# Jun-CEN/Open-World-Semantic-Segmentation

Hardware: AMD Instinct MI355X
Metric: images/sec train-step, DeepLabV3+R101 768x768 bs=16; % HBM & MFMA roofline (higher is better)
Workload: dtype f16x2

## Files before the change

include/dmlnet_hip.h:

```cpp
#ifndef DMLNET_HIP_H
#define DMLNET_HIP_H

#include <stdint.h>

#ifdef __cplusplus
extern "C" {
#endif

#define DML_ABI_VERSION 6

enum { DML_F32 = 0, DML_BF16 = 1 };
enum { DML_EINVAL = -1, DML_EALIGN = -2, DML_EUNSUPPORTED = -3 };

int dml_abi_version(void);
const char* dml_target_arch(void);

typedef struct DmlConvDesc {
    const void* x;
    const void* w;
    void* y;
    const float* bias;
    float* stats;
    int32_t B, Hi, Wi, C, ldx;
    int32_t Ho, Wo, N, ldy;
// ... 45 lines not shown
                 int32_t layout, float* work, int32_t amax_known, void* stream);

typedef struct DmlH2Desc {
    const float* x;
    void* planes;
    float* work;
    int64_t rows, plane_stride;
    int32_t C, ld, ldp, layout;
} DmlH2Desc;
int dml_h2_split_table(const DmlH2Desc* table_device, int count, void* stream);

typedef struct DmlWgradDesc {
    const void* x;
    const void* dy;
    float* dw;
    int32_t B, Hi, Wi, C, ldx;
    int32_t Ho, Wo, N, ldy;
    int32_t R, S, stride, dil, pad;
    int32_t dtype;
    int32_t splitk;
    int32_t Cm;
    float* ws;
    int64_t ws_elems;
    int32_t f32_split;
    int32_t reserved;
    const void* x_planes;
    const void* dy_planes;
    const float* x_unscale;
    const float* dy_unscale;
    int64_t x_plane_stride, dy_plane_stride;
} DmlWgradDesc;

int dml_conv_wgrad(const DmlWgradDesc* d, void* stream);

int dml_conv_wgrad_group_eligible(const DmlWgradDesc* d);
int dml_conv_wgrad_group(const DmlWgradDesc* const* descs, int n, float* ws, int64_t ws_elems, void* stream);

int dml_prep_weight(const float* w_master, void* w, void* wt, int N, int RS, int Cm, int Cp, int dtype,
                    void* stream);
typedef struct DmlPrepDesc {
    const float* src;
    void* w;
    void* wt;
    int32_t N, RS, Cm, Cp;
    int32_t w_tiled, wt_tiled;
} DmlPrepDesc;
int dml_prep_weights(const DmlPrepDesc* descs_device, int count, int dtype, void* stream);
int dml_unpad_wgrad(const float* src, float* dst, int N, int RS, int Cm, int Cp, void* stream);
int dml_bias_grad(const void* dy, float* db, int64_t M, int N, int ldy, int dtype, void* stream);
int dml_bias_grad_ws(const void* dy, float* db, int64_t M, int N, int ldy, int dtype, float* ws, int64_t ws_elems, void* stream);

int dml_pack_input(const float* x_nchw, void* y_nhwc, int B, int C, int H, int W, int Cp, int dtype,
                   void* stream);
int dml_pack_input_s2d(const float* x_nchw, float* x2, int B, int C, int H, int W, void* stream);
int dml_s2d_weights(const float* w, float* w2, int N, int k, int C, void* stream);
int dml_gather_taps(const float* src, float* dst, int rows, int taps_src, int n, int ntaps, int t0, int t1, int t2, int t3,
                    void* stream);
int dml_s2d_wgrad(const float* dw2, float* dw, int N, int k, int C, void* stream);

int dml_bn_finalize(float* partials, int64_t M, int N, int stat_rows, const float* gamma, const float* beta,
                    float* running_mean, float* running_var, float momentum, float eps,
                    float* scale, float* shift, float* save_mean, float* save_invstd, void* stream);
int dml_bn_moments(float* partials, int64_t M, int N, int stat_rows, double* moments, void* stream);
int dml_bn_finalize_moments(const double* moments, int ranks, int64_t M_each, int N, const float* gamma,
                            const float* beta, float* running_mean, float* running_var, float momentum,
                            float eps, float* scale, float* shift, float* save_mean, float* save_invstd,
// ... 258 lines not shown
```

open-world-semantic-segmentation_amd/csrc/bn.hip:

```cpp
#include "common.h"
#include <cstdlib>

namespace {

struct Moments {
    double n, mean, m2;
};
__device__ __forceinline__ void merge(Moments& a, double nb, double meanb, double m2b) {
    if (nb <= 0.0) return;
    const double n = a.n + nb;
    const double d = meanb - a.mean;
    a.mean += d * (nb / n);
    a.m2 += m2b + d * d * (a.n * nb / n);
    a.n = n;
}

constexpr int FIN_CH = 4, FIN_SL = 64;
__device__ __forceinline__ double shfl_xor_f64(double v, int mask) {
    const long long b = __double_as_longlong(v);
    const int lo = __shfl_xor((int)(b & 0xffffffffll), mask), hi = __shfl_xor((int)(b >> 32), mask);
    return __longlong_as_double(((long long)hi << 32) | (unsigned int)lo);
}

__device__ __forceinline__ float h2_words_max(const float* __restrict__ words, float* sh4) {
// ... 1197 lines not shown
            const uint32_t am = *reinterpret_cast<const uint32_t*>(argmax + o);
#pragma unroll
            for (int u = 0; u < 2; ++u) {
                const int r = 2 * by + u - (2 * yo - 1);
                if (r < 0 || r > 2) continue;
#pragma unroll
                for (int t = 0; t < 2; ++t) {
                    const int s = 2 * bx + t - (2 * xo - 1);
                    if (s < 0 || s > 2) continue;
#pragma unroll
                    for (int q = 0; q < 4; ++q) acc[u][t][q] += (((am >> (q * 8)) & 0xffu) == (uint32_t)(r * 3 + s)) ? g[q] : 0.f;
                }
            }
        }
    }
#pragma unroll
    for (int u = 0; u < 2; ++u) {
#pragma unroll
        for (int t = 0; t < 2; ++t) {
            const int yi = 2 * by + u, xi = 2 * bx + t;
            if (yi >= H || xi >= W) continue;
            const uint32_t bits = mask[(((int64_t)b * H + yi) * W + xi) * (C / 4) + cv];
#pragma unroll
            for (int q = 0; q < 4; ++q) acc[u][t][q] = ((bits >> q) & 1u) != 0 ? acc[u][t][q] : 0.f;
        }
    }
}

__device__ __forceinline__ void stem_pixel_grad(const float* __restrict__ dp, const uint8_t* __restrict__ argmax, uint32_t bits, int b,
                                                int yi, int xi, int C, int Ho, int Wo, int cv, float (&acc)[4]) {
#pragma unroll
    for (int q = 0; q < 4; ++q) acc[q] = 0.f;
    const int by = yi >> 1, bx = xi >> 1, u = yi & 1, t = xi & 1;
#pragma unroll
    for (int dyo = 0; dyo < 2; ++dyo) {
        const int yo = by + dyo, r = u + 1 - 2 * dyo;
        if (yo >= Ho || r < 0) continue;
#pragma unroll
        for (int dxo = 0; dxo < 2; ++dxo) {
            const int xo = bx + dxo, sc = t + 1 - 2 * dxo;
            if (xo >= Wo || sc < 0) continue;
            const int64_t o = (((int64_t)b * Ho + yo) * Wo + xo) * C + cv * 4;
            float g[4];
            Vec16<float>::load(dp + o, g);
            const uint32_t am = *reinterpret_cast<const uint32_t*>(argmax + o);
#pragma unroll
            for (int q = 0; q < 4; ++q) acc[q] += (((am >> (q * 8)) & 0xffu) == (uint32_t)(r * 3 + sc)) ? g[q] : 0.f;
        }
    }
#pragma unroll
    for (int q = 0; q < 4; ++q) acc[q] = ((bits >> q) & 1u) != 0 ? acc[q] : 0.f;
}

__global__ __launch_bounds__(256) void stem_bwd_reduce_kernel(
    const float* __restrict__ dp, const uint8_t* __restrict__ argmax, const uint8_t* __restrict__ mask, const float* __restrict__ y,
    const float* __restrict__ save_mean, const float* __restrict__ save_invstd, float* __restrict__ partials, int B, int H, int W,
    int C, int ldy, int Ho, int Wo, int rows_per_block, int chv, int rt, uint32_t* __restrict__ gmax) {
    __shared__ float sh[256 * 2 * 4];
    uint32_t gmx = 0;
    const int NV = C / 4;
    const int64_t M = (int64_t)B * H * W;
    const int col = threadIdx.x % chv, rl = threadIdx.x / chv;
    const int v = blockIdx.y * chv + col;
    const bool active = rl < rt && v < NV;
    float sg[4], sgx[4];
#pragma unroll
    for (int q = 0; q < 4; ++q) { sg[q] = 0.f; sgx[q] = 0.f; }
    if (active) {
        const int c = v * 4;
        float mu[4], is[4];
#pragma unroll
        for (int q = 0; q < 4; ++q) { mu[q] = save_mean[c + q]; is[q] = save_invstd[c + q]; }
        const int64_t r0 = (int64_t)blockIdx.x * rows_per_block;
        const int64_t r1 = min(M, r0 + rows_per_block);
        constexpr int U = 2;
        for (int64_t m0 = r0 + rl; m0 < r1; m0 += (int64_t)rt * U) {
            float g[U][4], yy[U][4];
#pragma unroll
            for (int u = 0; u < U; ++u) {
                const int64_t m = m0 + (int64_t)u * rt;
                if (m < r1) {
// ... 537 lines not shown
```

open-world-semantic-segmentation_amd/csrc/conv_igemm.hip:

```cpp
#include "common.h"
#include "conv_choice.h"
#include <cstdlib>

namespace {

constexpr int BK = 32;
constexpr int NTHREADS = 256;

typedef __bf16 mfma_bf16x8 __attribute__((ext_vector_type(8)));

struct ConvArgs {
    const void* x;
    const void* w;
    void* y;
    const float* bias;
    float* stats;
    int B, Hi, Wi, C, ldx;
    int Ho, Wo, N, ldy;
    int R, S, stride, dil, pad;
    int M, Ktot;
    int y_f32, accum;
    int nblk_n, nblk_m;
    FastDiv div_wo, div_howo, div_c;
    float* unused0_;
// ... 2193 lines not shown
        mm(0, 2); split_store(y_reg[1], Ys, lds_off(1)); split_store(x_reg[1], Xs, lds_off(1)); load_row(t + 2, 1);
        mm(1, 1); split_store(y_reg[2], Ys, lds_off(2)); split_store(x_reg[2], Xs, lds_off(2)); load_row(t + 2, 2);
        mm(1, 0); split_store(y_reg[3], Ys, lds_off(3)); split_store(x_reg[3], Xs, lds_off(3)); load_row(t + 2, 3);
        mm(0, 1);
        mm(0, 0);
#pragma unroll
        for (int q = 0; q < 64; ++q) {
            __builtin_amdgcn_sched_group_barrier(0x008, 1, 0);
            __builtin_amdgcn_sched_group_barrier(0x002, LIN ? 3 : 4, 0);
            __builtin_amdgcn_sched_group_barrier(0x200, 1, 0);
            if (q % 8 == 7) __builtin_amdgcn_sched_group_barrier(0x020, 1, 0);
        }
        __syncthreads();
    }
#pragma unroll
    for (int i = 0; i < NT; ++i)
#pragma unroll
        for (int q = 0; q < 4; ++q) {
            const int n = n0 + wn * 64 + i * 16 + lq * 4 + q;
            if (n >= a.N) continue;
#pragma unroll
            for (int j = 0; j < MT; ++j) {
                const int k = kc0 + wk * 64 + j * 16 + lr;
                if (k < a.Ktot) {
                    if (a.ws != nullptr)
                        a.ws[((int64_t)split * a.N + n) * a.Ktot + k] = acc[i][j][q];
                    else
                        atomicAdd(a.dw + (int64_t)n * a.Ktot + k, acc[i][j][q]);
                }
            }
        }
}

constexpr int WGW_NST = 3, WGW_NLD = 3;
constexpr int WGW_TN = 128, WGW_TK = 256;
constexpr int WGW_YROW = WGW_TN * 2, WGW_XROW = WGW_TK * 2;
constexpr int WGW_YPL = 32 * WGW_YROW, WGW_XPL = 32 * WGW_XROW;
constexpr int WGW_SB = 2 * WGW_YPL + 2 * WGW_XPL;

template <bool LIN, int LW>
__device__ __forceinline__ void wgrad_ws_loader(const WgradArgs& a, const uint32_t x_bytes, const uint32_t dy_bytes, char* smem,
                                                uint32_t* ready, uint32_t* consumed, const int lane, const int nitems, const int ntile) {
    constexpr int NLD = WGW_NLD, NST = WGW_NST, NG = 24, MYG = NG / NLD;
    constexpr uint32_t OOB = 0x80000000u;
    const u32x4_ws rs_x = ws_make_rsrc(a.x_planes, x_bytes + a.x_plane_bytes), rs_y = ws_make_rsrc(a.dy_planes, dy_bytes + a.dy_plane_bytes);
    const uint32_t lds0 = (uint32_t)(uintptr_t)smem;
    const int tiles_total = (a.M + BK - 1) / BK;
    uint32_t g = 0, pub = 0;
    for (int item = xcd_remap(blockIdx.x, gridDim.x); item < nitems; item += (int)gridDim.x) {
        const int split = item / ntile, tile_id = item - split * ntile;
        const int blk_n = tile_id % a.nblk_n, blk_k = tile_id / a.nblk_n;
        const int n0 = blk_n * WGW_TN, kc0 = blk_k * WGW_TK;
        const int tile_beg = split * a.slab_tiles, tile_end = min(tiles_total, tile_beg + a.slab_tiles);
        const int m_end = min(a.M, tile_end * BK);
        int row[MYG], colb[MYG], dyo[MYG], dxo[MYG];
        bool cok[MYG];
#pragma unroll
        for (int q = 0; q < MYG; ++q) {
            const int gi = q * NLD + LW;
            if (gi < 8) {
                row[q] = gi * 4 + (lane >> 4);
                const int gch = (lane & 15) ^ (2 * (row[q] & 7));
                const int n = n0 + gch * 8;
                cok[q] = n < a.N;
                colb[q] = n * 2;
                dyo[q] = dxo[q] = 0;
// ... 903 lines not shown
    switch (c.family) {
    case cc::WGRAD_BIG:
        hipLaunchKernelGGL(conv_wgrad_big_kernel<WGRAD_DEPTH>, grid, block, 0, st, a, c.x_bytes, c.dy_bytes);
        break;
    case cc::WGRAD_WS:
        if (c.lin) hipLaunchKernelGGL(conv_wgrad_ws_kernel<true>, grid, block, 0, st, a, c.x_bytes, c.dy_bytes, c.nitems);
        else hipLaunchKernelGGL(conv_wgrad_ws_kernel<false>, grid, block, 0, st, a, c.x_bytes, c.dy_bytes, c.nitems);
        break;
    case cc::WGRAD_H2:
        if (c.lin) hipLaunchKernelGGL(conv_wgrad_h2_kernel<true>, grid, block, 0, st, a, c.x_bytes, c.dy_bytes);
        else hipLaunchKernelGGL(conv_wgrad_h2_kernel<false>, grid, block, 0, st, a, c.x_bytes, c.dy_bytes);
        break;
    case cc::WGRAD_N64:
        hipLaunchKernelGGL(conv_wgrad_n64_kernel, grid, block, 0, st, a);
        break;
    case cc::WGRAD_X3:
        if (c.lin) hipLaunchKernelGGL(conv_wgrad_x3_kernel<true>, grid, block, 0, st, a, c.x_bytes, c.dy_bytes);
        else hipLaunchKernelGGL(conv_wgrad_x3_kernel<false>, grid, block, 0, st, a, c.x_bytes, c.dy_bytes);
        break;
    default:
        if (c.elem_bytes == 2) hipLaunchKernelGGL(conv_wgrad_kernel<bf16_t>, grid, block, 0, st, a);
        else hipLaunchKernelGGL(conv_wgrad_kernel<float>, grid, block, 0, st, a);
        break;
    }
    for (int i = 0; i < c.nreduce; ++i) {
        const cc::ReduceLaunch& r = c.reduce[i];
        hipLaunchKernelGGL(wgrad_reduce_kernel, dim3(r.grid_x, r.grid_y), dim3(r.block), 0, st, d->ws, d->dw, r.splits, c.nrs, c.cm, d->C,
                           r.slab_stride, r.fold_only);
    }
    DML_LAUNCH_CHECK();
    return 0;
}

extern "C" int dml_conv_wgrad_group_eligible(const DmlWgradDesc* d) { return cc::wgrad_big_eligible(d, true) ? 1 : 0; }

extern "C" int dml_conv_wgrad_group(const DmlWgradDesc* const* descs, int n, float* ws, int64_t ws_elems, void* stream) {
    cc::WgradGroupChoice c;
    const int rc = cc::wgrad_group_choose(descs, n, ws, ws_elems, &c);
    if (rc) return rc;
    WgradGroup g;
    ReduceGroup r;
    g.njobs = r.njobs = n;
    g.start[0] = 0;
    for (int j = 0; j < n; ++j) {
        const DmlWgradDesc* d = descs[j];
        WgradArgs& a = g.job[j];
        fill_wgrad_args(a, d, false);
        a.nblk_n = c.nblk_n[j]; a.nblk_k = c.nblk_k[j]; a.slab_tiles = c.slab_tiles[j];
        a.ws = ws + c.ws_off[j];
        g.xb[j] = c.x_bytes[j]; g.yb[j] = c.dy_bytes[j];
        g.start[j + 1] = c.start[j + 1];
        r.ws[j] = a.ws; r.dw[j] = d->dw; r.splits[j] = c.splitk[j]; r.Cm[j] = c.cm[j]; r.Cp[j] = d->C;
        r.NRS[j] = c.nrs[j];
    }
    hipStream_t st = static_cast<hipStream_t>(stream);
    hipLaunchKernelGGL(conv_wgrad_group_kernel<WGRAD_DEPTH>, dim3(c.grid), dim3(c.block), 0, st, g);
    hipLaunchKernelGGL(wgrad_reduce_group_kernel, dim3(c.rgrid_x, c.rgrid_y), dim3(c.rblock), 0, st, r);
    DML_LAUNCH_CHECK();
    return 0;
}
```

open-world-semantic-segmentation_amd/csrc/plan_exec.hip:

```cpp
#include "common.h"

#include <cstring>
#include <tuple>
#include <utility>

namespace {

template <class T> struct Unpack {
    static T get(uint64_t w) {
        if constexpr (std::is_pointer<T>::value) {
            return reinterpret_cast<T>(static_cast<uintptr_t>(w));
        } else if constexpr (std::is_same<T, float>::value) {
            const uint32_t lo = (uint32_t)w;
            float f;
            std::memcpy(&f, &lo, 4);
            return f;
        } else if constexpr (std::is_same<T, double>::value) {
            double d;
            std::memcpy(&d, &w, 8);
            return d;
        } else {
            return static_cast<T>(static_cast<int64_t>(w));
        }
    }
};

template <class R, class... Args, size_t... I>
int invoke(R (*f)(Args...), const uint64_t* w, void* st, std::index_sequence<I...>) {
    using Tup = std::tuple<Args...>;
    return (int)f(Unpack<std::tuple_element_t<I, Tup>>::get(w[I])..., st);
}
template <class R, class... Args> int thunk_call(R (*f)(Args...), const uint64_t* w, void* st) {
    return invoke(f, w, st, std::make_index_sequence<sizeof...(Args) - 1>{});
}
template <class R, class... Args> constexpr int arity(R (*)(Args...)) { return (int)sizeof...(Args) - 1; }

struct Entry {
    const char* name;
    int (*run)(const uint64_t*, void*);
    int nargs;
};

#define DML_ENTRY(fn) {#fn, [](const uint64_t* w, void* st) -> int { return thunk_call(&fn, w, st); }, arity(&fn)}

const Entry kEntries[] = {
    DML_ENTRY(dml_conv_igemm),
    DML_ENTRY(dml_conv_wgrad),
    DML_ENTRY(dml_conv_wgrad_group),
    DML_ENTRY(dml_prep_weight),
    DML_ENTRY(dml_prep_weights),
    DML_ENTRY(dml_unpad_wgrad),
    DML_ENTRY(dml_bias_grad),
    DML_ENTRY(dml_bias_grad_ws),
    DML_ENTRY(dml_pack_input),
    DML_ENTRY(dml_pack_input_s2d),
    DML_ENTRY(dml_s2d_weights),
    DML_ENTRY(dml_s2d_wgrad),
    DML_ENTRY(dml_bn_finalize),
    DML_ENTRY(dml_bn_moments),
    DML_ENTRY(dml_bn_finalize_moments),
    DML_ENTRY(dml_bn_bwd_sums),
    DML_ENTRY(dml_bn_bwd_coef),
    DML_ENTRY(dml_bn_stats),
    DML_ENTRY(dml_bn_eval_coeffs),
    DML_ENTRY(dml_bn_eval_coeffs_table),
    DML_ENTRY(dml_bn_apply),
    DML_ENTRY(dml_bn_bwd_reduce),
    DML_ENTRY(dml_bn_bwd_finalize),
    DML_ENTRY(dml_bn_bwd_apply),
    DML_ENTRY(dml_maxpool3x3s2_fwd),
    DML_ENTRY(dml_maxpool3x3s2_bwd),
    DML_ENTRY(dml_global_avgpool_fwd),
    DML_ENTRY(dml_broadcast_hw),
    DML_ENTRY(dml_reduce_hw),
    DML_ENTRY(dml_reduce_hw_f32),
    DML_ENTRY(dml_avgpool_bwd_add),
    DML_ENTRY(dml_avgpool_bwd_set),
    DML_ENTRY(dml_bilinear_fwd),
    DML_ENTRY(dml_bilinear_bwd),
    DML_ENTRY(dml_proto_dist_fwd),
    DML_ENTRY(dml_upsample_dist_fwd),
// ... 131 lines not shown
```

open-world-semantic-segmentation_amd/dmlnet/_lib.py:

```python
from __future__ import annotations

import ctypes as C
import os

_HERE = os.path.dirname(os.path.abspath(__file__))
LIB_PATH = os.environ.get("DML_LIB_PATH") or os.path.join(_HERE, "libdmlnet_hip.so")

DML_F32, DML_BF16 = 0, 1
STAT_ROWS = 64
LOSS_BLOCKS = 2048
FOCAL_PARTIALS = 3 * 2048
DISTILL_PARTIALS = 2 * 2048
OPEN_SWEEP_SPAN = 2048
OPEN_SWEEP_MAX_BLOCKS = 512
OPEN_SWEEP_MAX_T, OPEN_SWEEP_MAX_CLASSES, OPEN_SWEEP_MAX_OUT = 12, 33, 8


def metric_work_doubles(K, C):
    return 2048 * (2 + K * (C + 1))


c_p = C.c_void_p
c_i = C.c_int
c_i64 = C.c_int64
# ... 66 lines not shown
                ("op", C.c_int32 * 3), ("factor", C.c_float * 3)]


class ResizeScale(C.Structure):
    _fields_ = [("out", c_p), ("hbounds", c_p), ("hcoef", c_p), ("vbounds", c_p), ("vcoef", c_p),
                ("Hs", C.c_int32), ("Ws", C.c_int32), ("kh", C.c_int32), ("kv", C.c_int32),
                ("band_rows", C.c_int32), ("lds_rows", C.c_int32)]


RESIZE_MAX_SCALES = 8


class PredictHead(C.Structure):
    _fields_ = [("e", c_p), ("C", C.c_int32), ("K", C.c_int32), ("ld", C.c_int32), ("novel_id", C.c_int32)]


PREDICT_MAX_HEADS = 4
REC_MAX_SCALES = 8


class ScaleWindow(C.Structure):
    _fields_ = [("hbounds", C.c_int32), ("hcoef", C.c_int32), ("vbounds", C.c_int32), ("vcoef", C.c_int32),
                ("lrow", C.c_int32), ("lcol", C.c_int32), ("kh", C.c_int32), ("kv", C.c_int32)]


_PROTOS = {
    "dml_abi_version": (c_i, []),
    "dml_target_arch": (C.c_char_p, []),
    "dml_conv_igemm": (c_i, [C.POINTER(ConvDesc), c_p]),
    "dml_conv_stat_rows": (c_i, [C.POINTER(ConvDesc)]),
    "dml_h2_split_table": (c_i, [c_p, c_i, c_p]),
    "dml_h2_split": (c_i, [c_p, c_i64, c_i, c_i, c_p, c_i64, c_i, c_i, c_p, c_i, c_p]),
    "dml_conv_wgrad": (c_i, [C.POINTER(WgradDesc), c_p]),
    "dml_prep_weight": (c_i, [c_p, c_p, c_p, c_i, c_i, c_i, c_i, c_i, c_p]),
    "dml_prep_weights": (c_i, [c_p, c_i, c_i, c_p]),
    "dml_unpad_wgrad": (c_i, [c_p, c_p, c_i, c_i, c_i, c_i, c_p]),
    "dml_bias_grad": (c_i, [c_p, c_p, c_i64, c_i, c_i, c_i, c_p]),
    "dml_bias_grad_ws": (c_i, [c_p, c_p, c_i64, c_i, c_i, c_i, c_p, c_i64, c_p]),
    "dml_pack_input": (c_i, [c_p, c_p, c_i, c_i, c_i, c_i, c_i, c_i, c_p]),
    "dml_pack_input_s2d": (c_i, [c_p, c_p, c_i, c_i, c_i, c_i, c_p]),
    "dml_s2d_weights": (c_i, [c_p, c_p, c_i, c_i, c_i, c_p]),
    "dml_s2d_wgrad": (c_i, [c_p, c_p, c_i, c_i, c_i, c_p]),
    "dml_gather_taps": (c_i, [c_p, c_p, c_i, c_i, c_i, c_i, c_i, c_i, c_i, c_i, c_p]),
    "dml_bn_finalize": (c_i, [c_p, c_i64, c_i, c_i, c_p, c_p, c_p, c_p, c_f, c_f, c_p, c_p, c_p, c_p, c_p]),
    "dml_bn_moments": (c_i, [c_p, c_i64, c_i, c_i, c_p, c_p]),
    "dml_bn_finalize_moments": (c_i, [c_p, c_i, c_i64, c_i, c_p, c_p, c_p, c_p, c_f, c_f, c_p, c_p, c_p, c_p, c_p]),
    "dml_bn_bwd_sums": (c_i, [c_p, c_i, c_i, c_p, c_p, c_p, c_p]),
    "dml_bn_bwd_coef": (c_i, [c_p, c_i64, c_i, c_p, c_p, c_p, c_p, c_p]),
    "dml_bn_stats": (c_i, [c_p, c_p, c_i64, c_i, c_i, c_i, c_p]),
    "dml_bn_eval_coeffs": (c_i, [c_p, c_p, c_p, c_p, c_f, c_p, c_p, c_i, c_p]),
    "dml_bn_eval_coeffs_table": (c_i, [c_p, c_i, c_p]),
    "dml_bn_apply": (c_i, [c_p, c_p, c_p, c_p, c_p, c_p, c_p, c_i64, c_i, c_i, c_i, c_i, c_i, c_i, c_f, C.c_uint64, c_p,
                           c_p, c_i64, c_i, c_p, c_i64, c_p, c_p]),
    "dml_bn_bwd_reduce": (c_i, [c_p, c_p, c_p, c_p, c_p, c_p, c_p, c_i64, c_i, c_i, c_i, c_i, c_i, c_f, c_i,
                                C.POINTER(c_i), c_p, c_p]),
    "dml_bn_bwd_finalize": (c_i, [c_p, c_i, c_i64, c_i, c_p, c_p, c_p, c_p, c_p, c_p, c_p]),
    "dml_bn_bwd_apply": (c_i, [c_p, c_p, c_p, c_p, c_p, c_p, c_p, c_i64, c_i, c_i, c_i, c_i, c_i, c_i, c_i, c_f,
                               c_i, c_i, c_p, c_p, c_i64, c_i, c_p, c_p]),
    "dml_bn_relu_maxpool3x3s2_fwd": (c_i, [c_p, c_p, c_p, c_p, c_p, c_p, c_p, c_p, c_i64, c_p, c_p, c_i, c_i, c_i, c_i, c_i, c_p]),
    "dml_stem_bn_bwd_reduce": (c_i, [c_p, c_p, c_p, c_p, c_p, c_p, c_p, c_i, c_i, c_i, c_i, c_i, C.POINTER(c_i), c_p, c_p]),
    "dml_stem_bn_bwd_apply": (c_i, [c_p, c_p, c_p, c_p, c_p, c_p, c_i, c_i, c_i, c_i, c_i, c_i, c_p, c_i64, c_i, c_p, c_p]),
    "dml_head_bn_bwd_reduce": (c_i, [c_p, c_p, c_p, c_p, c_p, c_p, c_p, c_i64, c_i, c_i, c_i, c_i, c_i, c_i, c_i,
                                     C.POINTER(c_i), c_p, c_p]),
    "dml_head_bn_bwd_apply": (c_i, [c_p, c_p, c_p, c_p, c_p, c_p, c_i64, c_i, c_i, c_i, c_i, c_i, c_i, c_i, c_i, c_p, c_i64,
                                    c_i, c_p, c_p]),
    "dml_h2_bound_bn": (c_i, [c_p, c_p, c_i, c_i64, c_f, c_p, c_p, c_p]),
# ... 113 lines not shown
```

open-world-semantic-segmentation_amd/dmlnet/engine.py:

```python
from __future__ import annotations

import ctypes as C
import itertools
import os
import struct
import weakref
from typing import List, Optional

import numpy as np
import torch
import torch.distributed as dist
import torch.nn as nn

from . import _lib, lazy_grad
from ._lib import DML_BF16, DML_F32, STAT_ROWS, ConvDesc, WgradDesc

_PAD_CIN = 8


class _S2DConv:

    def __init__(self, conv: nn.Conv2d, Ho: int, Wo: int):
        k, p = conv.kernel_size[0], conv.padding[0]
        self.real, self.k = conv, k
# ... 272 lines not shown
        self.device = engine.store.flat_p.device
        self.fwd: list = []
        self.bwd: list = []
        self.prep: list = []
        self.keep: list = []
        self.units: List[ConvUnit] = []
        self.momentum_slots = []
        self.seed_slots = []
        self.prepped_version = None
        self.param_last_op = {}
        self.prep_table = None
        self.side = {}
        self._side_events = None
        self._nat, self._ev_handles, self._ev_objs = {}, None, None
        self.drop_units = []
        self.sync = bool(engine.sync_bn and training and dist.is_available() and dist.is_initialized()
                         and dist.get_world_size(engine.sync_group) > 1)
        self.world = dist.get_world_size(engine.sync_group) if self.sync else 1
        self.last_dgrad = {}
        self.res_src = {}
        self.f32_split = int(engine.f32_split) if dtype == torch.float32 else 0
        self.prep_h2 = []
        self.prep_h2_table = None
        self.h2_slots = torch.zeros(1025 * 1024, dtype=torch.float32, device=self.device) if self.f32_split == 2 else None
        self.h2_used = 0
        self.h2_direct_on = os.environ.get("DML_H2_DIRECT", "1") != "0"
        self.direct_planes = []
        self.fuse_res_grad = os.environ.get("DML_FUSE_RES_GRAD", "1") != "0"
        self.res_planes_on = os.environ.get("DML_RES_PLANES", "1") != "0"
        self.fuse_bn_reduce = os.environ.get("DML_FUSE_BN_REDUCE", "1") != "0"
        self.fuse_bound = os.environ.get("DML_FUSE_BOUND", "1") != "0"
        self.s2_classes_on = os.environ.get("DML_S2_CLASSES", "1") != "0"
        self.fuse_stem_on = os.environ.get("DML_FUSE_STEM", "1") != "0"
        self.fuse_head_dgrad_on = os.environ.get("DML_FUSE_HEAD_DGRAD", "1") != "0"
        self.prep_overlap_on = os.environ.get("DML_PREP_OVERLAP", "1") != "0"
        self.ds_grad_from_dz = os.environ.get("DML_DS_GRAD_FROM_DZ", "1") != "0"
        self.prep_gather = []
        self._bound_words, self._bound_used = None, 0
        self.stage32 = training and dtype == torch.bfloat16 and os.environ.get("DML_GRAD_STAGE32", "0") == "1"
        self.tiled_weights = os.environ.get("DML_W_TILED", "1") != "0" and os.environ.get("DML_CONV_V1") is None
        self.fork_branches = os.environ.get("DML_FORK_BRANCHES", "1") != "0"
        self.ws_min_tiles = int(os.environ.get("DML_WS_MIN_TILES", "0"))
        self.scratch = torch.empty(max(B * H * W * 3 // 4 + 16384, 1100 * 2048 * 2 + 65536), dtype=torch.float32,
                                   device=self.device)
        self.sp = self.scratch.data_ptr()
        self.wgrad_ws = torch.empty(64 * (1 << 20) if training else 1, dtype=torch.float32, device=self.device)
        self.tail_ws = torch.empty(512 * 128 * 128 if training else 1, dtype=torch.float32, device=self.device)
        self.tail_cnt = torch.zeros(128, dtype=torch.int32, device=self.device)
        self.group_wgrad = os.environ.get("DML_GROUP_WGRAD", "1") != "0"
        self.group_tiles = int(os.environ.get("DML_GROUP_TILES", "17"))
        self._wg_pending = []
        self.build()
        self.bytes = sum(t.numel() * t.element_size() for t in self.keep if isinstance(t, torch.Tensor))

    class _Precision:
        def __init__(self, plan, dtype):
            self.plan, self.dtype = plan, dtype

        def __enter__(self):
            p = self.plan
            self.saved = (p.dtype, p.dt, p.es, p.vec)
            p.dtype, p.dt = self.dtype, _dt(self.dtype)
            p.es = 2 if self.dtype == torch.bfloat16 else 4
            p.vec = 16 // p.es
            return p

# ... 234 lines not shown
                taps = [r * kw + t for r in rs for t in ss]
                sub = self.fbuf(x.C * len(taps) * dy.C)
                self.prep_gather.append((wt.data_ptr(), sub.data_ptr(), x.C, kh * kw, dy.C, len(taps), *(taps + [0] * (4 - len(taps)))))
                self.prepped_version = None
                dsc = ConvDesc(x=dy.ptr, w=sub.data_ptr(), y=gx.ptr, bias=None, stats=None, B=dy.B, Hi=dy.H, Wi=dy.W, C=dy.C, ldx=dy.ld,
                               Ho=dy.H, Wo=dy.W, N=x.C, ldy=gx.ld, R=len(rs), S=len(ss), stride=1, dil=1, pad=(cy + p - rs[0]) // 2,
                               dtype=self.dt, y_f32=0, accum=accum, mode=1)
                dsc.pad_w_set, dsc.pad_w = 1, (cx + p - ss[0]) // 2
                dsc.sub_grid, dsc.sub_y, dsc.sub_x = 1, cy, cx
                dsc.f32_split = 2
                dsc.x_planes, dsc.x_plane_stride, dsc.x_unscale = xpl
                dsc.w_planes, dsc.w_plane_stride, dsc.w_unscale = self.h2_weight(sub, x.C, len(taps) * dy.C)
                dsc.ws_min_tiles = self.ws_min_tiles
                dsc.tail_ws, dsc.tail_ws_elems = self.tail_ws.data_ptr(), self.tail_ws.numel()
                dsc.tail_counters, dsc.tail_counters_len = self.tail_cnt.data_ptr(), self.tail_cnt.numel()
                self.keep.append(dsc)
                self.call(self.bwd, lib.dml_conv_igemm, C.byref(dsc))
                descs.append(dsc)
        x.root.grad_init = True
        prev = self.last_dgrad.pop(gx.ptr, None)
        if len(descs) == 4:
            self.last_dgrad[gx.ptr] = descs
        elif (len(descs) == 1 and accum and prev is not None and not isinstance(prev, list) and not prev.sub_grid
              and os.environ.get("DML_BNR_INC", "1") != "0"
              and prev.y == gx.ptr and prev.N == x.C and prev.ldy == gx.ld and prev.f32_split == 2 and not prev.res_dz):
            descs[0].bnr_inc = 1
            self.last_dgrad[gx.ptr] = [prev, descs[0]]

    def round_staged(self, x: Act):
        g = self.grad_of(x)
        assert x is x.root and g.ld == g.C and x.g32.ld == g.C
        self.call(self.bwd, self.lib.dml_convert_dtype, x.g32.ptr, g.ptr, g.M * g.C, DML_F32, DML_BF16)

    def conv_wgrad(self, x: Act, dy: Act, conv: nn.Conv2d, Cp: int, pad_rows: int = 0):
        kh, kw, s, d, p, Ho, Wo = self.conv_geom(conv, x)
        Cm = conv.in_channels
        gptr = self.e.store.grad_ptr_of(conv.weight)
        h2 = None
        if self.f32_split == 2 and self.dtype == torch.float32 and x.C % 8 == 0 and (pad_rows or conv.out_channels) % 8 == 0:
            h2 = self.h2_of(x, self.bwd) + self.h2_of(dy, self.bwd)
        first = len(self.bwd)
        Nw, tmp = conv.out_channels, None
        s2d = isinstance(conv, _S2DConv)
        if s2d:
            assert not pad_rows
            tmp = self.fbuf(Nw * kh * kw * Cm)
            self.call(self.bwd, self.lib.dml_fill_f32, tmp.data_ptr(), tmp.numel(), 0.0)
        if pad_rows and pad_rows != conv.out_channels:
            Nw = pad_rows
            tmp = self.fbuf(Nw * kh * kw * Cm)
            self.call(self.bwd, self.lib.dml_fill_f32, tmp.data_ptr(), tmp.numel(), 0.0)
        dsc = WgradDesc(x=x.ptr, dy=dy.ptr, dw=tmp.data_ptr() if tmp is not None else gptr, B=x.B, Hi=x.H, Wi=x.W, C=x.C,
                        ldx=x.ld, Ho=Ho, Wo=Wo,
                        N=Nw, ldy=dy.ld, R=kh, S=kw, stride=s, dil=d, pad=p, dtype=self.dt, splitk=0,
                        Cm=Cm, ws=self.wgrad_ws.data_ptr(), ws_elems=self.wgrad_ws.numel(),
                        f32_split=min(self.f32_split, 1) if self.dtype == torch.float32 else 0)
        if h2 is not None:
            dsc.f32_split = 2
            (dsc.x_planes, dsc.x_plane_stride, dsc.x_unscale, dsc.dy_planes, dsc.dy_plane_stride, dsc.dy_unscale) = h2
        self.keep.append(dsc)
        if tmp is None and self.group_wgrad and self.lib.dml_conv_wgrad_group_eligible(C.byref(dsc)):
            Ktot = kh * kw * x.C
            base = (Nw // 256) * ((Ktot + 255) // 256)
            self._wg_pending.append((dsc, conv, base))
            if sum(b for _, _, b in self._wg_pending) >= self.group_tiles or len(self._wg_pending) >= 12:
                self.flush_wgrad()
            return
        self.call(self.bwd, self.lib.dml_conv_wgrad, C.byref(dsc))
        if s2d:
            self.call(self.bwd, self.lib.dml_s2d_wgrad, tmp.data_ptr(), gptr, conv.out_channels, conv.k, conv.real.in_channels)
        elif tmp is not None:
            self.call(self.bwd, self.lib.dml_unpad_wgrad, tmp.data_ptr(), gptr, conv.out_channels, kh * kw, Cm, Cm)
        for i in range(first, len(self.bwd)):
            self.side[i] = (i == first)
        self.mark_grad(conv.weight)

    def flush_wgrad(self):
        pend, self._wg_pending = self._wg_pending, []
        if not pend:
            return
        arr = (C.c_void_p * len(pend))(*[C.addressof(d) for d, _, _ in pend])
        self.keep.append(arr)
        i = len(self.bwd)
        args = self.call(self.bwd, self.lib.dml_conv_wgrad_group, C.addressof(arr), len(pend), self.wgrad_ws.data_ptr(),
                         self.wgrad_ws.numel())
        args.meta = [d for d, _, _ in pend]
        self.side[i] = True
        for _, conv, _ in pend:
            self.param_last_op[self.e.store._index(conv.weight)] = i

    def mark_grad(self, p):
        self.param_last_op[self.e.store._index(p)] = len(self.bwd) - 1

    def cbr(self, x: Act, conv: nn.Conv2d, bn: nn.BatchNorm2d, relu=True, res: Optional[Act] = None,
            out: Optional[Act] = None, drop: Optional[nn.Dropout] = None, need_dgrad=True, planes_only=False,
            pool_fused=False) -> ConvUnit:
        lib, st = self.lib, self.e.store
        u = ConvUnit()
        u.conv, u.bn, u.x, u.relu, u.res, u.drop = conv, bn, x, relu, res, drop
        u.dtype = self.dtype
        u.Cp = x.C
# ... 196 lines not shown
        else:
            self.call(self.bwd, lib.dml_bn_bwd_finalize, sp, nblk, 0 if u.frozen else M, N, bn.weight.data_ptr(),
                      u.mean.data_ptr(), u.invstd.data_ptr(), st.grad_ptr_of(bn.weight),
                      st.grad_ptr_of(bn.bias), coef.data_ptr())
        self.mark_grad(bn.weight)
        self.mark_grad(bn.bias)
        pl = (None, 0, 0, None)
        if dy_direct:
            planes, work = dy.h2
            if not bound_done:
                self.call(self.bwd, lib.dml_h2_bound_bn_bwd, coef.data_ptr(), u.invstd.data_ptr(), N, M * self.world,
                          gwork.data_ptr(), work.data_ptr())
            pl = (planes.data_ptr(), M * N, N, work.data_ptr() + 4096)
        if de is not None:
            assert dy_direct
            self.call(self.bwd, lib.dml_head_bn_bwd_apply, de.ptr, de_w, u.y.ptr, mk, coef.data_ptr(), None if only else dy.ptr,
                      M, N, de_k, de.C, de.ld, N, u.y.ld, dy.ld, 1 if relu_eff else 0, *pl)
        else:
            a3 = self.call(self.bwd, lib.dml_bn_bwd_apply, dz.ptr, u.y.ptr, u.z.ptr, mk, coef.data_ptr(),
                           None if only else dy.ptr, dres.ptr if dres is not None else None, M, N, dz.ld, u.y.ld, u.z.ld, dy.ld,
                           dres.ld if dres is not None else 0, 1 if relu_eff else 0, 1.0,
                           1 if dres_accum else 0, self.dt, None if dy_direct else self.amax_of(dy), *pl)
            u.gscale_slots += ([(a1, 13)] if a1 is not None else []) + [(a3, 15)]
        if dres is not None:
            self.last_dgrad.pop(dres.ptr, None)
        self.conv_wgrad(u.x, dy, u.conv, u.Cp)
        if need_dgrad:
            self.conv_dgrad(dy, u.conv, u.wt, u.x, final=final)

    def stem_bwd_fused(self, u: ConvUnit, dp: Act, argmax):
        lib, st = self.lib, self.e.store
        N, M, bn, y = u.conv.out_channels, u.y.M, u.bn, u.y
        planes = u.x.C % 8 == 0 and N % 8 == 0
        gwork = None
        if planes:
            only = self.planes_fit(M, N) and self.planes_fit(u.x.root.M, u.x.root.ld)
            dy = self.h2_direct(y.B, y.H, y.W, N, fp32_too=not only)
            gwork = self.h2_work()
        else:
            only = False
            dy = self.new(y.B, y.H, y.W, N)
        u.dz, u.dy, u.up = None, dy, None
        coef = self.fbuf(4 * N)
        nblk = C.c_int(0)
        self.keep.append(nblk)
        self.call(self.bwd, lib.dml_stem_bn_bwd_reduce, dp.ptr, argmax.data_ptr(), u.mask.data_ptr(), y.ptr, u.mean.data_ptr(),
                  u.invstd.data_ptr(), self.sp, y.B, y.H, y.W, N, y.ld, C.byref(nblk),
                  gwork.data_ptr() if gwork is not None else None)
        pl = (None, 0, 0, None)
        if planes and self.fuse_bound:
            self.call(self.bwd, lib.dml_bn_bwd_finalize_bound, self.sp, nblk, M, N, bn.weight.data_ptr(), u.mean.data_ptr(),
                      u.invstd.data_ptr(), st.grad_ptr_of(bn.weight), st.grad_ptr_of(bn.bias), coef.data_ptr(), M,
                      gwork.data_ptr(), dy.h2[1].data_ptr(), self.bound_state())
        else:
            self.call(self.bwd, lib.dml_bn_bwd_finalize, self.sp, nblk, M, N, bn.weight.data_ptr(), u.mean.data_ptr(),
                      u.invstd.data_ptr(), st.grad_ptr_of(bn.weight), st.grad_ptr_of(bn.bias), coef.data_ptr())
            if planes:
                self.call(self.bwd, lib.dml_h2_bound_bn_bwd, coef.data_ptr(), u.invstd.data_ptr(), N, M, gwork.data_ptr(),
                          dy.h2[1].data_ptr())
        self.mark_grad(bn.weight)
        self.mark_grad(bn.bias)
        if planes:
            pl = (dy.h2[0].data_ptr(), M * N, N, dy.h2[1].data_ptr() + 4096)
        self.call(self.bwd, lib.dml_stem_bn_bwd_apply, dp.ptr, argmax.data_ptr(), u.mask.data_ptr(), y.ptr, coef.data_ptr(),
                  None if only else dy.ptr, y.B, y.H, y.W, N, y.ld, dy.ld, *pl)
        self.conv_wgrad(u.x, dy, u.conv, u.Cp)

    def block_fwd(self, x: Act, blk: nn.Module, out_planes_only=False):
        n1, n2, n3 = blk.conv1.out_channels, blk.conv2.out_channels, blk.conv3.out_channels
        kk = blk.conv2.kernel_size[0] * blk.conv2.kernel_size[1]
        u1 = self.cbr(x, blk.conv1, blk.bn1, planes_only=self.h2_ok(n1, n2, kk))
        u2 = self.cbr(u1.z, blk.conv2, blk.bn2, planes_only=self.h2_ok(n2, n3, 1))
        ud = None
        if blk.downsample is not None:
            ud = self.cbr(x, blk.downsample[0], blk.downsample[1], relu=False)
            idt = ud.z
        else:
            idt = x
        u3 = self.cbr(u2.z, blk.conv3, blk.bn3, relu=True, res=idt, planes_only=out_planes_only)
        return (x, u1, u2, u3, ud)

    def block_bwd(self, rec):
        xb, u1, u2, u3, ud = rec
        dz = self.grad_of(u3.z)
        ud_from_dz = False
        if ud is not None:
            ud_from_dz = (self.ds_grad_from_dz and u3.relu and u3.mask is not None and u3.drop is None and not ud.relu
                          and ud.drop is None and ud.z is ud.z.root and ud.conv.out_channels == u3.conv.out_channels)
            if ud_from_dz:
                self.unit_bwd(u3, dz, dres=None)
            else:
                dres = self.grad_of(ud.z)
                self.unit_bwd(u3, dz, dres=dres, dres_accum=False)
                ud.z.grad_init = True
        elif (self.fuse_res_grad and not xb.root.grad_init and xb is xb.root
              and u3.relu and u3.mask is not None and u3.drop is None and xb.C % 8 == 0 and xb.C > 32
# ... 783 lines not shown
```

Before: 210.6.

## Fuse stem BN-backward apply and maxpool-grad into stem weight-gradient kernel

Adds a dedicated stem wgrad kernel that rebuilds dy on the fly from the pooled gradient, argmax, ReLU mask, BN output and BN coefficients. It splits dy into three bf16 planes in LDS and runs the 4x4 s2d stem wgrad GEMM on MFMA. This removes the separate stem BN apply kernel and the write and re-read of the full-resolution dy tensor. It also reshapes the stem pixel-grad helper to issue all four window loads before accumulating, with no branches. The cost is a specialized kernel with extra gather loads per row and a narrow eligibility check; other shapes fall back to the old path.

```diff
diff --git a/include/dmlnet_hip.h b/include/dmlnet_hip.h
--- a/include/dmlnet_hip.h
+++ b/include/dmlnet_hip.h
@@ -101,6 +101,9 @@
 } DmlWgradDesc;
 
 int dml_conv_wgrad(const DmlWgradDesc* d, void* stream);
+
+int dml_stem_wgrad(const DmlWgradDesc* d, const void* dp, const uint8_t* argmax, const uint8_t* mask, const void* y, const float* coef,
+                   void* stream);
 
 int dml_conv_wgrad_group_eligible(const DmlWgradDesc* d);
 int dml_conv_wgrad_group(const DmlWgradDesc* const* descs, int n, float* ws, int64_t ws_elems, void* stream);
diff --git a/open-world-semantic-segmentation_amd/csrc/bn.hip b/open-world-semantic-segmentation_amd/csrc/bn.hip
--- a/open-world-semantic-segmentation_amd/csrc/bn.hip
+++ b/open-world-semantic-segmentation_amd/csrc/bn.hip
@@ -1253,21 +1253,23 @@
 #pragma unroll
     for (int q = 0; q < 4; ++q) acc[q] = 0.f;
     const int by = yi >> 1, bx = xi >> 1, u = yi & 1, t = xi & 1;
-#pragma unroll
-    for (int dyo = 0; dyo < 2; ++dyo) {
+    float g[4][4];
+    uint32_t am[4], code[4];
+#pragma unroll
+    for (int w = 0; w < 4; ++w) {
+        const int dyo = w >> 1, dxo = w & 1;
         const int yo = by + dyo, r = u + 1 - 2 * dyo;
-        if (yo >= Ho || r < 0) continue;
-#pragma unroll
-        for (int dxo = 0; dxo < 2; ++dxo) {
-            const int xo = bx + dxo, sc = t + 1 - 2 * dxo;
-            if (xo >= Wo || sc < 0) continue;
-            const int64_t o = (((int64_t)b * Ho + yo) * Wo + xo) * C + cv * 4;
-            float g[4];
-            Vec16<float>::load(dp + o, g);
-            const uint32_t am = *reinterpret_cast<const uint32_t*>(argmax + o);
-#pragma unroll
-            for (int q = 0; q < 4; ++q) acc[q] += (((am >> (q * 8)) & 0xffu) == (uint32_t)(r * 3 + sc)) ? g[q] : 0.f;
-        }
+        const int xo = bx + dxo, sc = t + 1 - 2 * dxo;
+        const bool ok = (yo < Ho) & (r >= 0) & (xo < Wo) & (sc >= 0);
+        const int64_t o = (ok ? (((int64_t)b * Ho + yo) * Wo + xo) * C : (int64_t)0) + cv * 4;
+        Vec16<float>::load(dp + o, g[w]);
+        am[w] = *reinterpret_cast<const uint32_t*>(argmax + o);
+        code[w] = ok ? (uint32_t)(r * 3 + sc) : 0x100u;
+    }
+#pragma unroll
+    for (int w = 0; w < 4; ++w) {
+#pragma unroll
+        for (int q = 0; q < 4; ++q) acc[q] += (((am[w] >> (q * 8)) & 0xffu) == code[w]) ? g[w][q] : 0.f;
     }
 #pragma unroll
     for (int q = 0; q < 4; ++q) acc[q] = ((bits >> q) & 1u) != 0 ? acc[q] : 0.f;
diff --git a/open-world-semantic-segmentation_amd/csrc/conv_igemm.hip b/open-world-semantic-segmentation_amd/csrc/conv_igemm.hip
--- a/open-world-semantic-segmentation_amd/csrc/conv_igemm.hip
+++ b/open-world-semantic-segmentation_amd/csrc/conv_igemm.hip
@@ -2249,6 +2249,190 @@
         }
 }
 
+struct StemGradArgs {
+    const float* dp;
+    const uint8_t* argmax;
+    const uint8_t* mask;
+    const float* y;
+    const float* coef;
+    int Hp, Wp;
+    uint32_t dp_bytes, am_bytes, mask_bytes, y_bytes;
+};
+
+__global__ __launch_bounds__(NTHREADS) __attribute__((amdgpu_waves_per_eu(2))) void stem_wgrad_kernel(
+    const WgradArgs a, const StemGradArgs s, const uint32_t x_bytes) {
+    constexpr int SUB = 528, PLY = 4 * SUB, PLX = 12 * SUB;
+    constexpr int MT = 3, NT = 4;
+    constexpr int N = 64, KTOT = 192, CIN = 12, TAPS = 4;
+    constexpr uint32_t OOB = 0x80000000u;
+    __shared__ __attribute__((aligned(16))) bf16_t smem[3 * PLY + 3 * PLX + 8 * N];
+    bf16_t* const Ys = smem;
+    bf16_t* const Xs = smem + 3 * PLY;
+    float* const cfs = reinterpret_cast<float*>(smem + 3 * PLY + 3 * PLX);
+
+    const int tid = threadIdx.x, lane = tid & 63, wave = tid >> 6;
+    const int split = xcd_remap(blockIdx.x, gridDim.x);
+    const __amdgpu_buffer_rsrc_t rs_x = __builtin_amdgcn_make_buffer_rsrc(const_cast<void*>(a.x), 0, (int)x_bytes, 0x00020000);
+    const __amdgpu_buffer_rsrc_t rs_y = __builtin_amdgcn_make_buffer_rsrc(const_cast<float*>(s.y), 0, (int)s.y_bytes, 0x00020000);
+    const __amdgpu_buffer_rsrc_t rs_dp = __builtin_amdgcn_make_buffer_rsrc(const_cast<float*>(s.dp), 0, (int)s.dp_bytes, 0x00020000);
+    const __amdgpu_buffer_rsrc_t rs_am = __builtin_amdgcn_make_buffer_rsrc(const_cast<uint8_t*>(s.argmax), 0, (int)s.am_bytes, 0x00020000);
+    const __amdgpu_buffer_rsrc_t rs_mk = __builtin_amdgcn_make_buffer_rsrc(const_cast<uint8_t*>(s.mask), 0, (int)s.mask_bytes, 0x00020000);
+    const int c16 = tid & 15, r16 = tid >> 4;
+    int x_dy[3], x_dx[3], x_delta[3];
+#pragma unroll
+    for (int g = 0; g < 3; ++g) {
+        const int kc = g * 64 + c16 * 4, tap = kc / CIN, xc = kc - tap * CIN;
+        x_dy[g] = tap / TAPS - a.pad;
+        x_dx[g] = tap % TAPS - a.pad;
+        x_delta[g] = ((x_dy[g] * a.Wi + x_dx[g]) * a.ldx + xc) * 4;
+    }
+    const int tile_beg = split * a.slab_tiles;
+    const int tiles_total = (a.M + BK - 1) / BK;
+    const int tile_end = min(tiles_total, tile_beg + a.slab_tiles);
+
+    typedef unsigned int u32x4_t __attribute__((ext_vector_type(4)));
+    u32x4_t x_reg[6], y_reg[2];
+    u32x4_t dp_reg[2][4];
+    uint32_t am_reg[2][4], mk_reg[2], code[2];
+    cfs[tid] = s.coef[tid];
+    auto load_rows = [&](int t, int h) {
+        const int m = t * BK + r16 + h * 16;
+        const bool mv = (t < tile_end) & (m < a.M);
+        const uint32_t b = fdiv((uint32_t)m, a.div_howo);
+        const uint32_t rem = (uint32_t)m - b * (uint32_t)(a.Ho * a.Wo);
+        const uint32_t yo = fdiv(rem, a.div_wo);
+        const uint32_t xo = rem - yo * (uint32_t)a.Wo;
+        const uint32_t xb = (uint32_t)(((int)b * a.Hi + (int)yo) * a.Wi + (int)xo) * (uint32_t)a.ldx * 4u;
+#pragma unroll
+        for (int g = 0; g < 3; ++g) {
+            const bool xv = mv & ((unsigned)((int)yo + x_dy[g]) < (unsigned)a.Hi) & ((unsigned)((int)xo + x_dx[g]) < (unsigned)a.Wi);
+            x_reg[h * 3 + g] = __builtin_amdgcn_raw_buffer_load_b128(rs_x, (int)(xv ? xb + (uint32_t)x_delta[g] : OOB), 0, 0);
+        }
+        const uint32_t yo_b = ((uint32_t)m * (uint32_t)a.ldy + (uint32_t)(c16 * 4)) * 4u;
+        y_reg[h] = __builtin_amdgcn_raw_buffer_load_b128(rs_y, (int)(mv ? yo_b : OOB), 0, 0);
+        {
+            mk_reg[h] = __builtin_amdgcn_raw_buffer_load_b8(rs_mk, (int)(mv ? (uint32_t)m * 16u + (uint32_t)c16 : OOB), 0, 0);
+            const int by = (int)yo >> 1, bx = (int)xo >> 1, u = (int)yo & 1, v = (int)xo & 1;
+            uint32_t cd = 0;
+#pragma unroll
+            for (int w = 0; w < 4; ++w) {
+                const int dyo = w >> 1, dxo = w & 1;
+                const int yp = by + dyo, xp = bx + dxo, r = u + 1 - 2 * dyo, sc = v + 1 - 2 * dxo;
+                const bool wv = mv & (yp < s.Hp) & (xp < s.Wp) & (r >= 0) & (sc >= 0);
+                const uint32_t o = (uint32_t)((((int)b * s.Hp + yp) * s.Wp + xp) * N + c16 * 4);
+                dp_reg[h][w] = __builtin_amdgcn_raw_buffer_load_b128(rs_dp, (int)(wv ? o * 4u : OOB), 0, 0);
+                am_reg[h][w] = __builtin_amdgcn_raw_buffer_load_b32(rs_am, (int)(wv ? o : OOB), 0, 0);
+                cd |= (wv ? (uint32_t)(r * 3 + sc) : 0xffu) << (8 * w);
+            }
+            code[h] = cd;
+        }
+    };
+    auto dy_of = [&](int h) -> u32x4_t {
+        const f32x4 cA = *reinterpret_cast<const f32x4*>(cfs + c16 * 4), cB = *reinterpret_cast<const f32x4*>(cfs + N + c16 * 4);
+        const f32x4 cC = *reinterpret_cast<const f32x4*>(cfs + 2 * N + c16 * 4), cM = *reinterpret_cast<const f32x4*>(cfs + 3 * N + c16 * 4);
+        const uint32_t row_ok = (code[h] & 0xffu) != 0xffu ? 0xffffffffu : 0u;
+        u32x4_t o;
+#pragma unroll
+        for (int q = 0; q < 4; ++q) {
+            float g = 0.f;
+#pragma unroll
+            for (int w = 0; w < 4; ++w)
+                g += ((am_reg[h][w] >> (8 * q)) & 0xffu) == ((code[h] >> (8 * w)) & 0xffu) ? __uint_as_float(dp_reg[h][w][q]) : 0.f;
+            g = ((mk_reg[h] >> q) & 1u) != 0 ? g : 0.f;
+            const float v = cC[q] + __builtin_fmaf(cA[q], g, cB[q] * (__uint_as_float(y_reg[h][q]) - cM[q]));
+            o[q] = __float_as_uint(v) & row_ok;
+        }
+        return o;
+    };
+    auto split_store = [&](const u32x4_t v, bf16_t* plane0, const int pl, int off) {
+        const float x[4] = {__uint_as_float(v[0]), __uint_as_float(v[1]), __uint_as_float(v[2]), __uint_as_float(v[3])};
+        uint32_t h[2], m[2], l[2];
+#pragma unroll
+        for (int e = 0; e < 2; ++e) {
+            h[e] = pack_bf16x2(x[2 * e], x[2 * e + 1]);
+            const float r0 = x[2 * e] - __uint_as_float(h[e] << 16), r1 = x[2 * e + 1] - __uint_as_float(h[e] & 0xffff0000u);
+            m[e] = pack_bf16x2(r0, r1);
+            const float s0 = r0 - __uint_as_float(m[e] << 16), s1 = r1 - __uint_as_float(m[e] & 0xffff0000u);
+            l[e] = pack_bf16x2(s0, s1);
+        }
+        *reinterpret_cast<uint2*>(plane0 + off) = make_uint2(h[0], h[1]);
+        *reinterpret_cast<uint2*>(plane0 + pl + off) = make_uint2(m[0], m[1]);
+        *reinterpret_cast<uint2*>(plane0 + 2 * pl + off) = make_uint2(l[0], l[1]);
+    };
+    auto lds_off = [&](int h, int sub) {
+        const int row = r16 + h * 16;
+        const int prow_ = (row & 0x13) | (((row >> 3) & 1) << 2) | (((row >> 2) & 1) << 3);
+        return (sub + (c16 >> 2)) * SUB + prow_ * 16 + (c16 & 3) * 4;
+    };
+    auto store_y = [&](int h) { split_store(dy_of(h), Ys, PLY, lds_off(h, 0)); };
+    auto store_x = [&](int h, int g) { split_store(x_reg[h * 3 + g], Xs, PLX, lds_off(h, g * 4)); };
+
+    f32x4 acc[NT][MT];
+#pragma unroll
+    for (int i = 0; i < NT; ++i)
+#pragma unroll
+        for (int j = 0; j < MT; ++j) acc[i][j] = (f32x4){0.f, 0.f, 0.f, 0.f};
+    load_rows(tile_beg, 0);
+    load_rows(tile_beg, 1);
+    __syncthreads();
+#pragma unroll
+    for (int h = 0; h < 2; ++h) {
+        store_y(h);
+#pragma unroll
+        for (int g = 0; g < 3; ++g) store_x(h, g);
+    }
+    __syncthreads();
+    load_rows(tile_beg + 1, 0);
+    load_rows(tile_beg + 1, 1);
+    const int lr = lane & 15, lq = lane >> 4;
+    const int p_lo = ((lr >> 2) | ((lq & 1) << 2) | ((lq >> 1) << 4)) * 16 + (lr & 3) * 4;
+    const int p_hi = p_lo + 8 * 16;
+    const bf16_t* xs = Xs + wave * MT * SUB;
+    for (int t = tile_beg; t < tile_end; ++t) {
+        mfma_bf16x8 af[3][NT], bfr[3][MT];
+#pragma unroll
+        for (int p = 0; p < 3; ++p) {
+#pragma unroll
+            for (int i = 0; i < NT; ++i) {
+                const bf16x4 lo = lds_tr16_b64(Ys + p * PLY + i * SUB + p_lo);
+                const bf16x4 hi = lds_tr16_b64(Ys + p * PLY + i * SUB + p_hi);
+                bf16x8 v = {lo[0], lo[1], lo[2], lo[3], hi[0], hi[1], hi[2], hi[3]};
+                af[p][i] = __builtin_bit_cast(mfma_bf16x8, v);
+            }
+#pragma unroll
+            for (int j = 0; j < MT; ++j) {
+                const bf16x4 lo = lds_tr16_b64(xs + p * PLX + j * SUB + p_lo);
+                const bf16x4 hi = lds_tr16_b64(xs + p * PLX + j * SUB + p_hi);
+                bf16x8 v = {lo[0], lo[1], lo[2], lo[3], hi[0], hi[1], hi[2], hi[3]};
+                bfr[p][j] = __builtin_bit_cast(mfma_bf16x8, v);
+            }
+        }
+        __syncthreads();
+        auto mm = [&](int py, int px) {
+#pragma unroll
+            for (int i = 0; i < NT; ++i)
+#pragma unroll
+                for (int j = 0; j < MT; ++j)
+                    acc[i][j] = __builtin_amdgcn_mfma_f32_16x16x32_bf16(af[py][i], bfr[px][j], acc[i][j], 0, 0, 0);
+        };
+        mm(2, 0); store_y(0); store_x(0, 0); store_x(0, 1); store_x(0, 2); load_rows(t + 2, 0);
+        mm(0, 2);
+        mm(1, 1); store_y(1); store_x(1, 0); store_x(1, 1); store_x(1, 2); load_rows(t + 2, 1);
+        mm(1, 0);
+        mm(0, 1);
+        mm(0, 0);
+        __syncthreads();
+    }
+#pragma unroll
+    for (int i = 0; i < NT; ++i)
+#pragma unroll
+        for (int q = 0; q < 4; ++q) {
+            const int n = i * 16 + lq * 4 + q;
+#pragma unroll
+            for (int j = 0; j < MT; ++j) a.ws[((int64_t)split * N + n) * KTOT + wave * (MT * 16) + j * 16 + lr] = acc[i][j][q];
+        }
+}
+
 constexpr int WGW_NST = 3, WGW_NLD = 3;
 constexpr int WGW_TN = 128, WGW_TK = 256;
 constexpr int WGW_YROW = WGW_TN * 2, WGW_XROW = WGW_TK * 2;
@@ -3218,6 +3402,44 @@
     return 0;
 }
 
+extern "C" int dml_stem_wgrad(const DmlWgradDesc* d, const void* dp, const uint8_t* argmax, const uint8_t* mask, const void* y,
+                              const float* coef, void* stream) {
+    if (!d || !d->x || !d->dw || !dp || !argmax || !mask || !y || !coef) return DML_EINVAL;
+    if (d->B <= 0 || d->Hi <= 0 || d->Wi <= 0 || d->Ho <= 0 || d->Wo <= 0 || d->pad < 0) return DML_EINVAL;
+    if (d->dtype != DML_F32 || d->f32_split != 1 || d->N != 64 || d->R != 4 || d->S != 4 || d->C != 12 || d->stride != 1 || d->dil != 1 ||
+        !d->ws)
+        return DML_EUNSUPPORTED;
+    if ((cc::addr(d->x) & 15) || (cc::addr(y) & 15) || (cc::addr(dp) & 15) || (cc::addr(argmax) & 3) || (cc::addr(d->ws) & 3) ||
+        (cc::addr(coef) & 3))
+        return DML_EALIGN;
+    DmlWgradDesc dd = *d;
+    dd.dy = y;
+    cc::WgradChoice c;
+    const int rc = cc::wgrad_choose(&dd, &c);
+    if (rc) return rc;
+    if (c.family != cc::WGRAD_X3 || c.lin || !c.use_ws || c.nblk_n != 1 || c.nblk_k != 2) return DML_EUNSUPPORTED;
+    WgradArgs a;
+    fill_wgrad_args(a, &dd, false);
+    a.nblk_n = 1; a.nblk_k = 1; a.slab_tiles = c.slab_tiles;
+    a.ws = d->ws;
+    a.dy = nullptr;
+    StemGradArgs s{};
+    s.dp = static_cast<const float*>(dp); s.argmax = argmax; s.mask = mask; s.y = static_cast<const float*>(y); s.coef = coef;
+    s.Hp = (d->Ho - 1) / 2 + 1; s.Wp = (d->Wo - 1) / 2 + 1;
+    const int64_t pooled = (int64_t)d->B * s.Hp * s.Wp * 64;
+    s.dp_bytes = (uint32_t)(pooled * 4); s.am_bytes = (uint32_t)pooled;
+    s.mask_bytes = (uint32_t)((int64_t)a.M * 16); s.y_bytes = c.dy_bytes;
+    hipStream_t st = static_cast<hipStream_t>(stream);
+    hipLaunchKernelGGL(stem_wgrad_kernel, dim3(c.splitk), dim3(NTHREADS), 0, st, a, s, c.x_bytes);
+    for (int i = 0; i < c.nreduce; ++i) {
+        const cc::ReduceLaunch& r = c.reduce[i];
+        hipLaunchKernelGGL(wgrad_reduce_kernel, dim3(r.grid_x, r.grid_y), dim3(r.block), 0, st, d->ws, d->dw, r.splits, c.nrs, c.cm, d->C,
+                           r.slab_stride, r.fold_only);
+    }
+    DML_LAUNCH_CHECK();
+    return 0;
+}
+
 extern "C" int dml_conv_wgrad_group_eligible(const DmlWgradDesc* d) { return cc::wgrad_big_eligible(d, true) ? 1 : 0; }
 
 extern "C" int dml_conv_wgrad_group(const DmlWgradDesc* const* descs, int n, float* ws, int64_t ws_elems, void* stream) {
diff --git a/open-world-semantic-segmentation_amd/csrc/plan_exec.hip b/open-world-semantic-segmentation_amd/csrc/plan_exec.hip
--- a/open-world-semantic-segmentation_amd/csrc/plan_exec.hip
+++ b/open-world-semantic-segmentation_amd/csrc/plan_exec.hip
@@ -47,6 +47,7 @@
     DML_ENTRY(dml_conv_igemm),
     DML_ENTRY(dml_conv_wgrad),
     DML_ENTRY(dml_conv_wgrad_group),
+    DML_ENTRY(dml_stem_wgrad),
     DML_ENTRY(dml_prep_weight),
     DML_ENTRY(dml_prep_weights),
     DML_ENTRY(dml_unpad_wgrad),
diff --git a/open-world-semantic-segmentation_amd/dmlnet/_lib.py b/open-world-semantic-segmentation_amd/dmlnet/_lib.py
--- a/open-world-semantic-segmentation_amd/dmlnet/_lib.py
+++ b/open-world-semantic-segmentation_amd/dmlnet/_lib.py
@@ -122,6 +122,7 @@
     "dml_h2_split_table": (c_i, [c_p, c_i, c_p]),
     "dml_h2_split": (c_i, [c_p, c_i64, c_i, c_i, c_p, c_i64, c_i, c_i, c_p, c_i, c_p]),
     "dml_conv_wgrad": (c_i, [C.POINTER(WgradDesc), c_p]),
+    "dml_stem_wgrad": (c_i, [C.POINTER(WgradDesc), c_p, c_p, c_p, c_p, c_p, c_p]),
     "dml_prep_weight": (c_i, [c_p, c_p, c_p, c_i, c_i, c_i, c_i, c_i, c_p]),
     "dml_prep_weights": (c_i, [c_p, c_i, c_i, c_p]),
     "dml_unpad_wgrad": (c_i, [c_p, c_p, c_i, c_i, c_i, c_i, c_p]),
diff --git a/open-world-semantic-segmentation_amd/dmlnet/engine.py b/open-world-semantic-segmentation_amd/dmlnet/engine.py
--- a/open-world-semantic-segmentation_amd/dmlnet/engine.py
+++ b/open-world-semantic-segmentation_amd/dmlnet/engine.py
@@ -328,6 +328,7 @@
         self.fuse_bound = os.environ.get("DML_FUSE_BOUND", "1") != "0"
         self.s2_classes_on = os.environ.get("DML_S2_CLASSES", "1") != "0"
         self.fuse_stem_on = os.environ.get("DML_FUSE_STEM", "1") != "0"
+        self.fuse_stem_wgrad_on = os.environ.get("DML_FUSE_STEM_WGRAD", "1") != "0"
         self.fuse_head_dgrad_on = os.environ.get("DML_FUSE_HEAD_DGRAD", "1") != "0"
         self.prep_overlap_on = os.environ.get("DML_PREP_OVERLAP", "1") != "0"
         self.ds_grad_from_dz = os.environ.get("DML_DS_GRAD_FROM_DZ", "1") != "0"
@@ -628,7 +629,7 @@
         assert x is x.root and g.ld == g.C and x.g32.ld == g.C
         self.call(self.bwd, self.lib.dml_convert_dtype, x.g32.ptr, g.ptr, g.M * g.C, DML_F32, DML_BF16)
 
-    def conv_wgrad(self, x: Act, dy: Act, conv: nn.Conv2d, Cp: int, pad_rows: int = 0):
+    def conv_wgrad(self, x: Act, dy: Act, conv: nn.Conv2d, Cp: int, pad_rows: int = 0, stem_src=None):
         kh, kw, s, d, p, Ho, Wo = self.conv_geom(conv, x)
         Cm = conv.in_channels
         gptr = self.e.store.grad_ptr_of(conv.weight)
@@ -646,7 +647,7 @@
             Nw = pad_rows
             tmp = self.fbuf(Nw * kh * kw * Cm)
             self.call(self.bwd, self.lib.dml_fill_f32, tmp.data_ptr(), tmp.numel(), 0.0)
-        dsc = WgradDesc(x=x.ptr, dy=dy.ptr, dw=tmp.data_ptr() if tmp is not None else gptr, B=x.B, Hi=x.H, Wi=x.W, C=x.C,
+        dsc = WgradDesc(x=x.ptr, dy=None if stem_src else dy.ptr, dw=tmp.data_ptr() if tmp is not None else gptr, B=x.B, Hi=x.H, Wi=x.W, C=x.C,
                         ldx=x.ld, Ho=Ho, Wo=Wo,
                         N=Nw, ldy=dy.ld, R=kh, S=kw, stride=s, dil=d, pad=p, dtype=self.dt, splitk=0,
                         Cm=Cm, ws=self.wgrad_ws.data_ptr(), ws_elems=self.wgrad_ws.numel(),
@@ -662,7 +663,11 @@
             if sum(b for _, _, b in self._wg_pending) >= self.group_tiles or len(self._wg_pending) >= 12:
                 self.flush_wgrad()
             return
-        self.call(self.bwd, self.lib.dml_conv_wgrad, C.byref(dsc))
+        if stem_src:
+            dp, argmax, mask, coef = stem_src
+            self.call(self.bwd, self.lib.dml_stem_wgrad, C.byref(dsc), dp, argmax, mask, dy.ptr, coef)
+        else:
+            self.call(self.bwd, self.lib.dml_conv_wgrad, C.byref(dsc))
         if s2d:
             self.call(self.bwd, self.lib.dml_s2d_wgrad, tmp.data_ptr(), gptr, conv.out_channels, conv.k, conv.real.in_channels)
         elif tmp is not None:
@@ -925,8 +930,12 @@
         lib, st = self.lib, self.e.store
         N, M, bn, y = u.conv.out_channels, u.y.M, u.bn, u.y
         planes = u.x.C % 8 == 0 and N % 8 == 0
+        in_wgrad = (self.fuse_stem_wgrad_on and not planes and isinstance(u.conv, _S2DConv) and u.conv.kernel_size == (4, 4)
+                    and u.x.C == 12 and N == 64 and self.f32_split >= 1)
         gwork = None
-        if planes:
+        if in_wgrad:
+            dy = None
+        elif planes:
             only = self.planes_fit(M, N) and self.planes_fit(u.x.root.M, u.x.root.ld)
             dy = self.h2_direct(y.B, y.H, y.W, N, fp32_too=not only)
             gwork = self.h2_work()
@@ -955,6 +964,9 @@
         self.mark_grad(bn.bias)
         if planes:
             pl = (dy.h2[0].data_ptr(), M * N, N, dy.h2[1].data_ptr() + 4096)
+        if in_wgrad:
+            self.conv_wgrad(u.x, y, u.conv, u.Cp, stem_src=(dp.ptr, argmax.data_ptr(), u.mask.data_ptr(), coef.data_ptr()))
+            return
         self.call(self.bwd, lib.dml_stem_bn_bwd_apply, dp.ptr, argmax.data_ptr(), u.mask.data_ptr(), y.ptr, coef.data_ptr(),
                   None if only else dy.ptr, y.B, y.H, y.W, N, y.ld, dy.ld, *pl)
         self.conv_wgrad(u.x, dy, u.conv, u.Cp)
```

Result: no change. 212.5 (median of 6 runs) (+0.9%).
